# sara-nl/2D-VQ-AE-2

Hardware: AMD Instinct MI355X
Metric: patches/sec (VQAE.forward: encoder -> VQ -> decoder) (higher is better)
Workload: dtype f32; 1 GPU; BASELINE configs[1] (cfg B): batch 256/GPU of 256x256x3 fp32 -> 32x32 codes, K=256, D=128, full forward; global_batch=256, parallelism=patch-sharded x1

## Files before the change

### 2d-vq-ae-2_amd/_lib.py

```python
import ctypes
import os
from ctypes import POINTER, Structure, c_char_p, c_double, c_float, c_int, c_int64, c_size_t, c_void_p

_HERE = os.path.dirname(os.path.abspath(__file__))
LIB_PATH = os.environ.get("VQAE_HIP_LIB") or os.path.join(_HERE, "libvqae_hip.so")

LAYOUT_NHWC, LAYOUT_NCHW = 0, 1
IDX_I64, IDX_U8, IDX_U16, IDX_I32 = 0, 1, 2, 3
PAD_NONE, PAD_CIRCULAR, PAD_ZEROS = 0, 1, 2
PRE_NONE, PRE_BIAS, PRE_BIAS_ELU_BIAS, PRE_CHANNEL_GATE = 0, 1, 2, 3
ACT_NONE, ACT_ELU, ACT_SILU = 0, 1, 2
DW_SAME, DW_DOWN, DW_UP = 0, 1, 2
MBT_ROWS, MBT_FIN_LANES = 256, 64
BLOCK_FIXUP, BLOCK_MBCONV = 0, 1
DT_F32, DT_BF16, DT_F16 = 0, 1, 2
MAX_PIXEL_LEVEL = 6
METRIC_NAMES = ("mse", "huber", "psnr", "ssim", "pred_min", "pred_max", "target_min", "target_max")
CLS_STATS_NAMES = ("tp", "fp", "fn", "tn", "n_valid", "loss_sum")
CE_STATS_K, CE_WEIGHT_SUM, CE_NLL_SUM, CE_SMOOTH_SUM, CE_N_BAD = 20, 16, 17, 18, 19
DTYPES = {"f32": DT_F32, "fp32": DT_F32, "float32": DT_F32, "bf16": DT_BF16, "bfloat16": DT_BF16,
          "f16": DT_F16, "fp16": DT_F16, "float16": DT_F16, "half": DT_F16}


def dtype_code(dt):
    if dt is None:
        return DT_F32
    if isinstance(dt, int):
        return dt
    name = str(dt).replace("torch.", "")
    try:
        return DTYPES[name]
    except KeyError:
        raise AssertionError(f"unsupported compute dtype {dt}")


class VqaeHipError(RuntimeError):
    pass


class ConvArgs(Structure):
    _fields_ = [("batch", c_int), ("in_h", c_int), ("in_w", c_int), ("cin", c_int), ("cout", c_int),
                ("ksize", c_int), ("stride", c_int), ("pad", c_int), ("pad_mode", c_int),
                ("pre_mode", c_int), ("pre_a", c_float), ("pre_b", c_float),
                ("has_scale", c_int), ("has_bias_s", c_int), ("has_act", c_int),
                ("scale", c_float), ("bias_s", c_float), ("act_a", c_float), ("act_b", c_float), ("dtype", c_int)]


class Config(Structure):
    _fields_ = [("in_channels", c_int), ("stem", c_int), ("n_down", c_int), ("n_pre", c_int), ("n_post", c_int),
                ("n_enc", c_int), ("num_embeddings", c_int), ("projection_dim", c_int),
                ("commitment_cost", c_float), ("compute_dtype", c_int),
                ("block_kind", c_int), ("expand_ratio", c_int), ("se_divisor", c_int), ("bn_eps", c_float)]


class Tensor(Structure):
    _fields_ = [("name", c_char_p), ("data", c_void_p), ("numel", c_int64)]


OPTIM_KINDS = {"adam": 0, "adamw": 1, "lamb": 2}
OPTIM_CHUNK, OPTIM_SMALL = 4096, 64


class ClassifierOptimConfig(Structure):
    _fields_ = [("kind", c_int), ("lr", c_double), ("beta1", c_double), ("beta2", c_double), ("eps", c_double),
                ("weight_decay", c_double), ("sam_rho", c_double), ("sam_adaptive", c_int)]


SYMBOLS = {
    "vqae_last_error": (c_char_p, []),
    "vqae_build_info": (c_char_p, []),
    "vqae_vq_workspace_bytes": (c_size_t, [c_int64, c_int, c_int]),
    "vqae_vq_forward_f32": (c_int, [c_void_p, c_void_p, c_int64, c_int, c_int, c_float, c_void_p, c_int, c_void_p,
                                    c_void_p, c_void_p, c_void_p, c_void_p]),
    "vqae_vq_forward_p_f32": (c_int, [c_void_p, c_void_p, c_int64, c_int, c_int, c_int, c_float, c_void_p, c_int, c_void_p,
                                      c_void_p, c_void_p, c_void_p, c_void_p]),
    "vqae_vq_projected_workspace_bytes": (c_size_t, [c_int64]),
    "vqae_vq_projected_f32": (c_int, [c_void_p, c_void_p, c_void_p, c_void_p, c_void_p, c_void_p, c_int64, c_int, c_int, c_int,
                                      c_float, c_int, c_void_p, c_int, c_void_p, c_void_p, c_void_p, c_void_p, c_void_p, c_void_p]),
    "vqae_vq_backward_f32": (c_int, [c_void_p, c_void_p, c_void_p, c_void_p, c_float, c_int64, c_int, c_void_p, c_void_p]),
    "vqae_vq_projected_backward_workspace_bytes": (c_size_t, [c_int64, c_int]),
    "vqae_vq_projected_backward_f32": (c_int, [c_void_p, c_void_p, c_void_p, c_void_p, c_void_p, c_void_p, c_void_p, c_int64,
                                               c_int, c_int, c_float, c_void_p, c_void_p, c_void_p, c_void_p, c_void_p,
                                               c_void_p, c_void_p]),
    "vqae_embed_code_f32": (c_int, [c_void_p, c_int, c_void_p, c_int64, c_int, c_int, c_void_p, c_void_p]),
    "vqae_vq_code_stats_f32": (c_int, [c_void_p, c_void_p, c_int, c_int64, c_int, c_int, c_void_p, c_void_p, c_void_p]),
    "vqae_vq_ema_update_f32": (c_int, [c_void_p, c_void_p, c_void_p, c_void_p, c_void_p, c_int, c_int, c_double, c_double,
                                       c_void_p, c_void_p]),
    "vqae_conv_packed_floats": (c_size_t, [c_int, c_int, c_int]),
    "vqae_conv_pack_weight_f32": (c_int, [c_void_p, c_int, c_int, c_int, c_void_p, c_void_p]),
    "vqae_conv2d_f32": (c_int, [POINTER(ConvArgs), c_void_p, c_void_p, c_void_p, c_void_p, c_void_p, c_void_p]),
    "vqae_conv2d_gated_f32": (c_int, [POINTER(ConvArgs), c_void_p, c_void_p, c_void_p, c_void_p, c_void_p, c_void_p,
                                      c_void_p]),
    "vqae_dw_partial_floats": (c_size_t, [c_int, c_int, c_int, c_int]),
    "vqae_dwconv_f32": (c_int, [c_void_p, c_void_p, c_void_p, c_int, c_int, c_int, c_int, c_int, c_int, c_void_p,
                                c_void_p, c_void_p]),
    "vqae_se_gate_f32": (c_int, [c_void_p, c_int, c_int, c_int, c_int, c_void_p, c_void_p, c_int, c_void_p, c_void_p,
                                 c_void_p, c_void_p]),
    "vqae_pixel_shuffle2_f32": (c_int, [c_void_p, c_int, c_int, c_int, c_int, c_void_p, c_void_p]),
    "vqae_fixup_same_supported": (c_int, [c_int, c_int, c_int]),
    "vqae_fixup_same_block_f32": (c_int, [c_void_p, c_void_p, c_void_p, c_void_p, c_void_p, c_int, c_int, c_int, c_int,
                                          POINTER(c_float), c_int, c_void_p]),
    "vqae_round_inplace_f32": (c_int, [c_void_p, c_int64, c_int, c_void_p]),
    "vqae_conv3x3_direct_f32": (c_int, [c_void_p, c_void_p, POINTER(c_float), POINTER(c_float), c_void_p, c_void_p,
                                        c_int, c_int, c_int, c_int, c_int, c_void_p, c_int, c_void_p]),
    "vqae_bicubic_up2_f32": (c_int, [c_void_p, c_int, c_int, c_int, c_int, c_float, c_void_p, c_void_p]),
    "vqae_nchw_to_nhwc_f32": (c_int, [c_void_p, c_int, c_int, c_int, c_int, c_void_p, c_void_p]),
    "vqae_nhwc_to_nchw_f32": (c_int, [c_void_p, c_int, c_int, c_int, c_int, c_void_p, c_void_p]),
    "vqae_label_maxpool_u8": (c_int, [c_void_p, c_int, c_int, c_int, c_int, c_void_p, c_void_p]),
    "vqae_stitch_tiles": (c_int, [c_void_p, c_int, c_void_p, c_int, c_int, c_int, c_void_p, c_int, c_int, c_int,
                                  c_void_p]),
    "vqae_unstitch_tiles": (c_int, [c_void_p, c_int, c_void_p, c_int, c_int, c_int, c_void_p, c_int, c_int, c_int,
                                    c_void_p]),
    "vqae_pixels_u8": (c_int, [c_void_p, c_int, c_int, c_int, c_int, c_void_p, POINTER(c_float), POINTER(c_float), c_void_p,
                               c_int, c_int, c_void_p]),
    "vqae_pixels_u8_level": (c_int, [c_void_p, c_int, c_int, c_int, c_int, c_int, c_void_p, POINTER(c_float), POINTER(c_float),
                                     c_void_p, c_int, c_int, c_void_p]),
    "vqae_cut_pixels_u8": (c_int, [c_void_p, c_int, c_int, c_int, c_void_p, c_int, c_int, c_int, c_int, c_int, c_int, c_void_p,
                                   c_void_p]),
    "vqae_pool_labels_u8": (c_int, [c_void_p, c_int, c_int, c_int, c_int, c_int, c_int, c_void_p, c_int, c_int, c_void_p]),
    "vqae_create": (c_int, [POINTER(Config), POINTER(Tensor), c_int, POINTER(c_void_p)]),
    "vqae_destroy": (None, [c_void_p]),
    "vqae_reserve": (c_int, [c_void_p, c_int, c_int, c_int]),
    "vqae_set_codebook": (c_int, [c_void_p, c_void_p]),
    "vqae_encode": (c_int, [c_void_p, c_void_p, c_int, c_int, c_int, c_int, c_void_p, c_int, c_void_p, c_void_p,
                            c_void_p]),
    "vqae_encode_u8": (c_int, [c_void_p, c_void_p, c_int, c_int, c_int, c_void_p, c_int, c_void_p, c_int, c_void_p,
                               c_void_p]),
    "vqae_encode_features": (c_int, [c_void_p, c_void_p, c_int, c_int, c_int, c_int, c_void_p, c_void_p]),
    "vqae_decode": (c_int, [c_void_p, c_void_p, c_int, c_int, c_int, c_int, c_void_p, c_void_p]),
    "vqae_decode_indices": (c_int, [c_void_p, c_void_p, c_int, c_int, c_int, c_int, c_int, c_void_p, c_void_p]),
    "vqae_decode_indices_u8": (c_int, [c_void_p, c_void_p, c_int, c_int, c_int, c_int, c_void_p, c_void_p, c_int, c_int,
                                       c_void_p]),
    "vqae_decode_indices_u8_levels": (c_int, [c_void_p, c_void_p, c_int, c_int, c_int, c_int, c_void_p, c_int, POINTER(c_int),
                                              POINTER(c_void_p), POINTER(c_int), POINTER(c_int), c_void_p]),
    "vqae_forward": (c_int, [c_void_p, c_void_p, c_int, c_int, c_int, c_int, c_void_p, c_void_p, c_int, c_void_p,
                             c_void_p]),
    "vqae_block_count": (c_int, [c_void_p, c_int]),
    "vqae_run_blocks": (c_int, [c_void_p, c_int, c_int, c_int, c_void_p, c_int, c_int, c_int, c_void_p, POINTER(c_int),
                                POINTER(c_int), c_void_p]),
    "vqae_block_route": (c_char_p, [c_void_p, c_int, c_int, c_int, c_int, c_int, c_int]),
    "vqae_recon_metrics_workspace_bytes": (c_size_t, [c_int, c_int, c_int, c_int]),
    "vqae_recon_metrics_f32": (c_int, [c_void_p, c_void_p, c_void_p, POINTER(c_float), POINTER(c_float), c_int, c_int, c_int,
                                       c_int, c_int, c_float, c_void_p, c_void_p, c_void_p]),
    "vqae_classifier_create": (c_int, [c_int, c_int, c_int, c_int, POINTER(Tensor), c_int, POINTER(c_void_p)]),
    "vqae_classifier_destroy": (None, [c_void_p]),
    "vqae_classifier_workspace_bytes": (c_size_t, [c_void_p, c_int, c_int, c_int]),
    "vqae_classifier_forward": (c_int, [c_void_p, c_void_p, c_int, c_int, c_int, c_int, c_void_p, c_void_p, c_void_p, c_float,
                                        c_void_p, c_void_p, c_void_p]),
    "vqae_classifier_update": (c_int, [c_void_p, POINTER(Tensor), c_int]),
    "vqae_classifier_grad_floats": (c_size_t, [c_void_p]),
    "vqae_classifier_train_workspace_bytes": (c_size_t, [c_void_p, c_int, c_int, c_int]),
    "vqae_classifier_loss_grad": (c_int, [c_void_p, c_void_p, c_int, c_int, c_int, c_int, c_void_p, c_void_p, c_float, c_int,
                                          c_void_p, c_void_p, c_void_p, c_void_p, c_void_p]),
    "vqae_classifier_optim_create": (c_int, [c_void_p, POINTER(ClassifierOptimConfig), POINTER(c_void_p)]),
    "vqae_classifier_optim_destroy": (None, [c_void_p]),
    "vqae_classifier_optim_set": (c_int, [c_void_p, POINTER(ClassifierOptimConfig)]),
    "vqae_classifier_optim_step": (c_int, [c_void_p, c_void_p, c_void_p]),
    "vqae_classifier_optim_sam_first": (c_int, [c_void_p, c_void_p, c_void_p]),
    "vqae_classifier_download": (c_int, [c_void_p, POINTER(c_void_p), c_void_p]),
    "vqae_classifier_image_floats": (c_size_t, [c_void_p]),
    "vqae_classifier_image": (c_int, [c_void_p, c_void_p, c_void_p]),
    "vqae_classifier_optim_export": (c_int, [c_void_p, c_void_p, c_void_p, POINTER(c_int64), c_void_p]),
    "vqae_classifier_optim_import": (c_int, [c_void_p, c_void_p, c_void_p, c_int64, c_void_p]),
    "vqae_classifier_ce_workspace_bytes": (c_size_t, [c_void_p, c_int, c_int, c_int]),
    "vqae_classifier_forward_ce": (c_int, [c_void_p, c_void_p, c_int, c_int, c_int, c_int, c_void_p, c_void_p, c_void_p, c_void_p,
                                           POINTER(c_float), c_float, c_void_p, c_void_p, c_void_p]),
    "vqae_classifier_ce_train_workspace_bytes": (c_size_t, [c_void_p, c_int, c_int, c_int]),
    "vqae_classifier_loss_grad_ce": (c_int, [c_void_p, c_void_p, c_int, c_int, c_int, c_int, c_void_p, POINTER(c_float), c_float,
                                             c_int, c_void_p, c_void_p, c_void_p, c_void_p, c_void_p]),
    "vqae_classifier_optim_create_ce": (c_int, [c_void_p, POINTER(ClassifierOptimConfig), POINTER(c_void_p)]),
    "vqae_optim_create": (c_int, [c_int, POINTER(c_int64), POINTER(c_int), c_int, POINTER(ClassifierOptimConfig),
                                  POINTER(c_void_p)]),
    "vqae_optim_destroy": (None, [c_void_p]),
    "vqae_optim_set": (c_int, [c_void_p, POINTER(ClassifierOptimConfig)]),
    "vqae_optim_step": (c_int, [c_void_p, POINTER(c_void_p), POINTER(c_void_p), c_void_p]),
    "vqae_optim_sam_first": (c_int, [c_void_p, POINTER(c_void_p), POINTER(c_void_p), c_void_p]),
    "vqae_optim_export": (c_int, [c_void_p, c_void_p, c_void_p, POINTER(c_int64), c_void_p]),
    "vqae_optim_import": (c_int, [c_void_p, c_void_p, c_void_p, POINTER(c_int64), c_void_p]),
    "vqae_fixup_train_workspace_bytes": (c_size_t, [c_int64]),
    "vqae_fixup_act_f32": (c_int, [c_void_p, c_void_p, c_void_p, c_int, c_int, c_int, c_int, c_int, c_int, c_void_p, c_void_p]),
    "vqae_fixup_act_backward_f32": (c_int, [c_void_p, c_void_p, c_void_p, c_int, c_int, c_int, c_int, c_int, c_int, c_void_p,
                                            c_void_p, c_void_p, c_void_p, c_void_p]),
    "vqae_fixup_out_f32": (c_int, [c_void_p, c_void_p, c_void_p, c_void_p, c_void_p, c_int64, c_void_p, c_void_p]),
    "vqae_fixup_out_backward_f32": (c_int, [c_void_p, c_void_p, c_void_p, c_int64, c_void_p, c_void_p, c_void_p, c_void_p,
                                            c_void_p, c_void_p]),
    "vqae_fixup_act_io": (c_int, [c_void_p, c_int, c_void_p, c_void_p, c_int, c_int, c_int, c_int, c_int, c_int, c_void_p, c_int,
                                  c_void_p]),
# ... 93 lines not shown
```

### 2d-vq-ae-2_amd/csrc/misc_kernels.hip

```cpp
#include "kernels.h"
#include "mfma.h"

namespace {


template <int CIN, int COUT>
__global__ __launch_bounds__(256)
void conv3x3_direct_kernel(const void* __restrict__ xin, int x_kind, Norm3 nrm, const float* __restrict__ w,
                           const float* __restrict__ bias, int B, int H, int W, float* __restrict__ y, int y_nchw,
                           int dt) {
    __shared__ float ws[9 * CIN * COUT + COUT];
    for (int i = threadIdx.x; i < 9 * CIN * COUT; i += 256) {
        const int co = i % COUT, ci = (i / COUT) % CIN, tap = i / (COUT * CIN);
        ws[i] = vqae::round_dt(w[((int64_t)co * CIN + ci) * 9 + tap], dt);
    }
    for (int i = threadIdx.x; i < COUT; i += 256) ws[9 * CIN * COUT + i] = vqae::round_dt(bias[i], dt);
    __syncthreads();

    const int64_t npix = (int64_t)B * H * W;
    const int64_t pix = (int64_t)blockIdx.x * 256 + threadIdx.x;
    if (pix >= npix) return;
    const int hw = H * W;
    const int b = (int)(pix / hw), rem = (int)(pix - (int64_t)b * hw);
    const int oy = rem / W, ox = rem - oy * W;
// ... 151 lines not shown
    if (i >= (int64_t)B * O * O) return;
    const int ox = (int)(i % O), oy = (int)((i / O) % O), b = (int)(i / ((int64_t)O * O));
    const int y0 = (oy * H) / O, y1 = ((oy + 1) * H + O - 1) / O;
    const int x0 = (ox * W) / O, x1 = ((ox + 1) * W + O - 1) / O;
    uint8_t m = 0;
    for (int yy = y0; yy < y1; ++yy)
        for (int xx = x0; xx < x1; ++xx) {
            const uint8_t v = lab[((int64_t)b * H + yy) * W + xx];
            m = v > m ? v : m;
        }
    y[i] = m;
}

template <typename TI, typename TO>
__global__ __launch_bounds__(256)
void stitch_kernel(const TI* __restrict__ tiles, const int32_t* __restrict__ rc, int64_t total, int th, int tw,
                   TO* __restrict__ grid, int gh, int gw) {
    const int64_t i = (int64_t)blockIdx.x * 256 + threadIdx.x;
    if (i >= total) return;
    const int x = (int)(i % tw), yy = (int)((i / tw) % th);
    const int64_t t = i / ((int64_t)tw * th);
    const int r = rc[2 * t], c = rc[2 * t + 1];
    const int64_t gy = (int64_t)r * th + yy, gx = (int64_t)c * tw + x;
    if (gy < gh && gx < gw) grid[gy * gw + gx] = (TO)tiles[i];
}

template <int CIN>
__global__ __launch_bounds__(256)
void ostem_rb_kernel(const float* __restrict__ x, const float* __restrict__ w, const float* __restrict__ bias, int B, int H, int W,
                     float* __restrict__ y, int y_nchw) {
    constexpr int QN = CIN / 4;
    typedef float f32x4_t __attribute__((ext_vector_type(4)));
    const int q = threadIdx.x % QN;
    f32x4_t wr[9][3];
#pragma unroll
    for (int tap = 0; tap < 9; ++tap)
#pragma unroll
        for (int co = 0; co < 3; ++co)
#pragma unroll
            for (int e = 0; e < 4; ++e) wr[tap][co][e] = w[((int64_t)co * CIN + 4 * q + e) * 9 + tap];
    const float b0 = bias[0], b1 = bias[1], b2 = bias[2];
    const int hw = H * W;
    const int64_t npix = (int64_t)B * hw;
    const int64_t stride = (int64_t)gridDim.x * (256 / QN);
    const int64_t trips = (npix + stride - 1) / stride;
    int64_t pix = (int64_t)blockIdx.x * (256 / QN) + threadIdx.x / QN;
    for (int64_t t = 0; t < trips; ++t, pix += stride) {
        const bool live = pix < npix;
        const int64_t pc = live ? pix : npix - 1;
        const int b = (int)(pc / hw), rem = (int)(pc - (int64_t)b * hw);
        const int oy = rem / W, ox = rem - oy * W;
        float a0 = 0.f, a1 = 0.f, a2 = 0.f;
#pragma unroll
        for (int tap = 0; tap < 9; ++tap) {
            const int iy = oy + tap / 3 - 1, ix = ox + tap % 3 - 1;
            const bool ok = iy >= 0 && iy < H && ix >= 0 && ix < W;
            const int64_t src = ((int64_t)b * hw + (ok ? (int64_t)iy * W + ix : rem)) * CIN + 4 * q;
            f32x4_t v = *reinterpret_cast<const f32x4_t*>(x + src);
            if (!ok) v = (f32x4_t){0.f, 0.f, 0.f, 0.f};
#pragma unroll
            for (int e = 0; e < 4; ++e) {
                a0 = __builtin_fmaf(v[e], wr[tap][0][e], a0);
                a1 = __builtin_fmaf(v[e], wr[tap][1][e], a1);
                a2 = __builtin_fmaf(v[e], wr[tap][2][e], a2);
            }
        }
#pragma unroll
        for (int off = 1; off < QN; off <<= 1) {
            a0 += __shfl_xor(a0, off);
            a1 += __shfl_xor(a1, off);
            a2 += __shfl_xor(a2, off);
        }
        if (live && q == 0) {
            a0 += b0; a1 += b1; a2 += b2;
            if (y_nchw) {
                y[((int64_t)b * 3 + 0) * hw + rem] = a0;
                y[((int64_t)b * 3 + 1) * hw + rem] = a1;
                y[((int64_t)b * 3 + 2) * hw + rem] = a2;
            } else {
                y[pix * 3 + 0] = a0; y[pix * 3 + 1] = a1; y[pix * 3 + 2] = a2;
            }
        }
    }
}

template <int CIN, int COUT>
int launch_direct(const void* x, int x_kind, const Norm3& nrm, const float* w, const float* bias, int B, int H, int W,
                  float* y, int y_nchw, int dt, hipStream_t stream) {
    const int64_t npix = (int64_t)B * H * W;
    conv3x3_direct_kernel<CIN, COUT><<<(unsigned)vqae::ceil_div(npix, 256), 256, 0, stream>>>(
        x, x_kind, nrm, w, bias, B, H, W, y, y_nchw, dt);
    VQAE_LAUNCH_CHECK();
    return VQAE_OK;
}

template <typename TI>
int stitch_out(const TI* tiles, const int32_t* rc, int64_t total, int th, int tw, void* grid, int gdt, int gh, int gw,
               hipStream_t stream) {
    const unsigned g = (unsigned)vqae::ceil_div(total, 256);
    switch (gdt) {
        case VQAE_IDX_I64: stitch_kernel<TI, int64_t><<<g, 256, 0, stream>>>(tiles, rc, total, th, tw, (int64_t*)grid, gh, gw); break;
        case VQAE_IDX_U8: stitch_kernel<TI, uint8_t><<<g, 256, 0, stream>>>(tiles, rc, total, th, tw, (uint8_t*)grid, gh, gw); break;
        case VQAE_IDX_U16: stitch_kernel<TI, uint16_t><<<g, 256, 0, stream>>>(tiles, rc, total, th, tw, (uint16_t*)grid, gh, gw); break;
        case VQAE_IDX_I32: stitch_kernel<TI, int32_t><<<g, 256, 0, stream>>>(tiles, rc, total, th, tw, (int32_t*)grid, gh, gw); break;
        default: return vqae::fail(VQAE_ERR_INVALID, "stitch: bad grid dtype %d", gdt);
    }
    VQAE_LAUNCH_CHECK();
    return VQAE_OK;
}


struct SmallK {
    const float* __restrict__ x;
    const float* __restrict__ w;
    const float* __restrict__ bias_vec;
    const float* residual;
    float* y;
    int H, W, Ho, Wo, cout;
    int64_t M;
    int pre_mode, has_scale, has_bias_s, has_act, dt;
    float pre_a, pre_b, scale, bias_s, act_a, act_b;
};

template <int KS>
__global__ __launch_bounds__(256)
void conv_small_k_kernel(const SmallK p) {
    constexpr int K = KS * KS * 8;
    __shared__ __attribute__((aligned(16))) float Wl[K * 64];
    const int cg4 = p.cout >> 2;
    for (int j = threadIdx.x; j < K * p.cout; j += 256) Wl[j] = p.w[(int64_t)(j % p.cout) * K + j / p.cout];
    __syncthreads();
    const int64_t i = (int64_t)blockIdx.x * 256 + threadIdx.x;
    if (i >= p.M * cg4) return;
    const int cg = (int)(i % cg4);
    const int64_t m = i / cg4;
    const int ox = (int)(m % p.Wo);
    const int64_t t = m / p.Wo;
    const int oy = (int)(t % p.Ho);
    const int64_t b = t / p.Ho;
    float v[K];
#pragma unroll
    for (int tap = 0; tap < KS * KS; ++tap) {
        const float4* src = reinterpret_cast<const float4*>(
            p.x + (((b * p.H + (int64_t)oy * KS + tap / KS) * p.W) + (int64_t)ox * KS + tap % KS) * 8);
        const float4 a = src[0], c = src[1];
        v[tap * 8 + 0] = a.x; v[tap * 8 + 1] = a.y; v[tap * 8 + 2] = a.z; v[tap * 8 + 3] = a.w;
        v[tap * 8 + 4] = c.x; v[tap * 8 + 5] = c.y; v[tap * 8 + 6] = c.z; v[tap * 8 + 7] = c.w;
    }
#pragma unroll
    for (int k = 0; k < K; ++k) {
        if (p.pre_mode != VQAE_PRE_NONE) {
            v[k] = v[k] + p.pre_a;
            if (p.pre_mode == VQAE_PRE_BIAS_ELU_BIAS) v[k] = vqae::elu_act(v[k]) + p.pre_b;
        }
        v[k] = vqae::round_dt(v[k], p.dt);
    }
    float out[4] = {0.f, 0.f, 0.f, 0.f};
#pragma unroll
    for (int k = 0; k < K; ++k) {
        const float4 wv = *reinterpret_cast<const float4*>(Wl + k * p.cout + 4 * cg);
        out[0] = __builtin_fmaf(v[k], wv.x, out[0]); out[1] = __builtin_fmaf(v[k], wv.y, out[1]);
        out[2] = __builtin_fmaf(v[k], wv.z, out[2]); out[3] = __builtin_fmaf(v[k], wv.w, out[3]);
    }
#pragma unroll
    for (int e = 0; e < 4; ++e) {
        float acc = out[e];
        if (p.bias_vec) acc = acc + p.bias_vec[4 * cg + e];
        acc = vqae::round_dt(acc, p.dt);
        if (p.has_scale) { acc = acc * p.scale; acc = acc + p.bias_s; }
        else if (p.has_bias_s) { acc = acc + p.bias_s; }
        out[e] = acc;
    }
    const int64_t o = m * p.cout + 4 * cg;
    if (p.residual) {
        const float4 r = *reinterpret_cast<const float4*>(p.residual + o);
        out[0] += r.x; out[1] += r.y; out[2] += r.z; out[3] += r.w;
    }
    if (p.has_act == VQAE_ACT_SILU) {
#pragma unroll
        for (int e = 0; e < 4; ++e) out[e] = out[e] / (1.0f + expf(-out[e]));
    } else if (p.has_act) {
#pragma unroll
        for (int e = 0; e < 4; ++e) out[e] = vqae::elu_act(out[e] + p.act_a) + p.act_b;
    }
    *reinterpret_cast<float4*>(p.y + o) = make_float4(out[0], out[1], out[2], out[3]);
}

}

namespace vqae {
bool conv_small_k_supported(const vqae_conv_args* a) {
    return a->cin == 8 && a->pad == 0 && a->ksize == a->stride && (a->ksize == 1 || a->ksize == 2) && a->cout % 4 == 0 &&
           a->cout <= 64 && a->pre_mode <= VQAE_PRE_BIAS_ELU_BIAS && a->in_h % a->ksize == 0 && a->in_w % a->ksize == 0;
}

int conv_small_k(const vqae_conv_args* a, const float* x, const float* w, const float* bias_vec, const float* residual,
                 float* y, hipStream_t stream) {
    SmallK p;
    p.x = x; p.w = w; p.bias_vec = bias_vec; p.residual = residual; p.y = y;
    p.H = a->in_h; p.W = a->in_w; p.Ho = a->in_h / a->ksize; p.Wo = a->in_w / a->ksize; p.cout = a->cout;
    p.M = (int64_t)a->batch * p.Ho * p.Wo;
    p.pre_mode = a->pre_mode; p.has_scale = a->has_scale; p.has_bias_s = a->has_bias_s; p.has_act = a->has_act; p.dt = a->dtype;
    p.pre_a = a->pre_a; p.pre_b = a->pre_b; p.scale = a->scale; p.bias_s = a->bias_s; p.act_a = a->act_a; p.act_b = a->act_b;
    const int64_t threads = p.M * (a->cout / 4);
    if (threads == 0) return VQAE_OK;
    VQAE_REQUIRE(ceil_div(threads, 256) < (1ll << 31), VQAE_ERR_UNSUPPORTED, "conv_small_k: too many pixels");
    const unsigned grid = (unsigned)ceil_div(threads, 256);
    if (a->ksize == 1) conv_small_k_kernel<1><<<grid, 256, 0, stream>>>(p);
    else conv_small_k_kernel<2><<<grid, 256, 0, stream>>>(p);
    VQAE_LAUNCH_CHECK();
    return VQAE_OK;
}

int conv3x3_direct(const void* x, int x_kind, const float* mean255, const float* inv_std255, const float* w,
                   const float* bias, int B, int H, int W, int cin, int cout, float* y, int y_nchw, int dt,
                   hipStream_t stream) {
    Norm3 nrm;
    for (int i = 0; i < 4; ++i) {
        nrm.mean[i] = (mean255 && i < 3) ? mean255[i] : 0.f;
        nrm.inv[i] = (inv_std255 && i < 3) ? inv_std255[i] : 1.f;
    }
    VQAE_REQUIRE(x && w && bias && y, VQAE_ERR_INVALID, "conv3x3_direct: null pointer");
    VQAE_REQUIRE(x_kind != 2 || cin == 3, VQAE_ERR_UNSUPPORTED, "conv3x3_direct: uint8 input needs cin == 3");
    if ((int64_t)B * H * W == 0) return VQAE_OK;
    static const bool no_rb = env_int("VQAE_NO_STEM_RB", 0) != 0;
    if (!no_rb && dt == VQAE_DT_F32) {
        if (cout == 3 && x_kind == 0 && (cin == 8 || cin == 16 || cin == 32)) {
            const int64_t npix = (int64_t)B * H * W;
            const unsigned grid = (unsigned)std::min<int64_t>(vqae::ceil_div(npix, 256 / (cin / 4)), 256 * 12);
            if (cin == 8) ostem_rb_kernel<8><<<grid, 256, 0, stream>>>((const float*)x, w, bias, B, H, W, y, y_nchw);
            else if (cin == 16) ostem_rb_kernel<16><<<grid, 256, 0, stream>>>((const float*)x, w, bias, B, H, W, y, y_nchw);
            else ostem_rb_kernel<32><<<grid, 256, 0, stream>>>((const float*)x, w, bias, B, H, W, y, y_nchw);
            VQAE_LAUNCH_CHECK();
            return VQAE_OK;
        }
    }
#define VQAE_DIRECT_CASE(CI, CO) \
    if (cin == CI && cout == CO) return launch_direct<CI, CO>(x, x_kind, nrm, w, bias, B, H, W, y, y_nchw, dt, stream);
    VQAE_DIRECT_CASE(3, 4) VQAE_DIRECT_CASE(3, 8) VQAE_DIRECT_CASE(3, 16) VQAE_DIRECT_CASE(3, 32) VQAE_DIRECT_CASE(3, 64)
    VQAE_DIRECT_CASE(4, 3) VQAE_DIRECT_CASE(8, 3) VQAE_DIRECT_CASE(16, 3) VQAE_DIRECT_CASE(32, 3) VQAE_DIRECT_CASE(64, 3)
#undef VQAE_DIRECT_CASE
    return fail(VQAE_ERR_UNSUPPORTED, "conv3x3_direct: unsupported channel pair %d -> %d", cin, cout);
}
}

extern "C" int vqae_conv3x3_direct_f32(const float* x, const uint8_t* x_u8, const float* mean255, const float* inv_std255,
                                       const float* w, const float* bias, int B, int H, int W, int cin, int cout,
                                       float* y, int dtype, void* stream) {
    VQAE_REQUIRE(dtype >= VQAE_DT_F32 && dtype <= VQAE_DT_F16, VQAE_ERR_INVALID, "conv3x3_direct: dtype %d", dtype);
    static const bool no16 = vqae::env_int("VQAE_NO_STEM16", 0) != 0;
    const int c0 = cin == 3 ? cout : (cout == 3 ? cin : 0);
    if (!no16 && dtype != VQAE_DT_F32 && c0 && (cin == 3) != (cout == 3) && vqae::stem16_supported(c0, H, W, dtype) && (cin == 3 || x)) {
        VQAE_REQUIRE((x || x_u8) && w && bias && y, VQAE_ERR_INVALID, "conv3x3_direct: null pointer");
        void* wbuf = nullptr;
        VQAE_HIP_CHECK(hipMallocAsync(&wbuf, vqae::stem16_weight_bytes(32), (hipStream_t)stream));
        int rc = vqae::stem16_pack_weight(w, cout, cin, dtype, wbuf, (hipStream_t)stream);
        if (rc == VQAE_OK)
            rc = cin == 3 ? vqae::istem16(x_u8 ? (const void*)x_u8 : (const void*)x, x_u8 ? 2 : 0, mean255, inv_std255, wbuf, bias, B, H, W,
                                          cout, y, dtype, (hipStream_t)stream)
                          : vqae::ostem16(x, wbuf, bias, B, H, W, cin, y, 0, dtype, (hipStream_t)stream);
        const hipError_t fe = hipFreeAsync(wbuf, (hipStream_t)stream);
        if (rc == VQAE_OK && fe != hipSuccess) return vqae::fail(VQAE_ERR_HIP, "conv3x3_direct: hipFreeAsync: %s", hipGetErrorString(fe));
        return rc;
    }
    if (x_u8)
        return vqae::conv3x3_direct(x_u8, 2, mean255, inv_std255, w, bias, B, H, W, cin, cout, y, 0, dtype, (hipStream_t)stream);
    return vqae::conv3x3_direct(x, 0, nullptr, nullptr, w, bias, B, H, W, cin, cout, y, 0, dtype, (hipStream_t)stream);
}

namespace {
__global__ void round_inplace_kernel(float* __restrict__ x, int64_t n, int dt) {
    const int64_t i = (int64_t)blockIdx.x * 256 + threadIdx.x;
    if (i < n) x[i] = vqae::round_dt(x[i], dt);
}
}

extern "C" int vqae_round_inplace_f32(float* x, int64_t n, int dtype, void* stream) {
    VQAE_REQUIRE(dtype >= VQAE_DT_F32 && dtype <= VQAE_DT_F16, VQAE_ERR_INVALID, "round_inplace: dtype %d", dtype);
    if (n == 0 || dtype == VQAE_DT_F32) return VQAE_OK;
    VQAE_REQUIRE(x, VQAE_ERR_INVALID, "round_inplace: null pointer");
    round_inplace_kernel<<<(unsigned)vqae::ceil_div(n, 256), 256, 0, (hipStream_t)stream>>>(x, n, dtype);
    VQAE_LAUNCH_CHECK();
    return VQAE_OK;
}

extern "C" int vqae_bicubic_up2_f32(const float* x, int B, int H, int W, int C, float pre_bias, float* y, void* stream_) {
    hipStream_t stream = (hipStream_t)stream_;
    VQAE_REQUIRE(x && y, VQAE_ERR_INVALID, "bicubic_up2: null pointer");
    VQAE_REQUIRE(C % 4 == 0, VQAE_ERR_UNSUPPORTED, "bicubic_up2: channels %d must be a multiple of 4", C);
    if ((int64_t)B * H * W == 0) return VQAE_OK;
    const int64_t total = (int64_t)B * (H + 1) * (W + 1) * (C / 4);
    const unsigned grid = (unsigned)std::min<int64_t>(vqae::ceil_div(total, 256), 256 * 64);
    bicubic_up2_kernel<<<grid, 256, 0, stream>>>((const float4*)x, B, H, W, C / 4, pre_bias, (float4*)y);
    VQAE_LAUNCH_CHECK();
    return VQAE_OK;
}

static int transpose_batched(const float* x, int B, int R, int S, float* y, hipStream_t stream) {
    if ((int64_t)B * R * S == 0) return VQAE_OK;
    VQAE_REQUIRE(B <= 65535, VQAE_ERR_UNSUPPORTED, "transpose: batch %d > 65535", B);
    dim3 grid((unsigned)vqae::ceil_div(S, 32), (unsigned)vqae::ceil_div(R, 32), (unsigned)B);
    transpose_kernel<<<grid, 256, 0, stream>>>(x, R, S, y);
    VQAE_LAUNCH_CHECK();
    return VQAE_OK;
}

extern "C" int vqae_nchw_to_nhwc_f32(const float* x, int B, int C, int H, int W, float* y, void* stream) {
    VQAE_REQUIRE(x && y, VQAE_ERR_INVALID, "nchw_to_nhwc: null pointer");
    return transpose_batched(x, B, C, H * W, y, (hipStream_t)stream);
}

extern "C" int vqae_nhwc_to_nchw_f32(const float* x, int B, int C, int H, int W, float* y, void* stream) {
    VQAE_REQUIRE(x && y, VQAE_ERR_INVALID, "nhwc_to_nchw: null pointer");
    return transpose_batched(x, B, H * W, C, y, (hipStream_t)stream);
}

extern "C" int vqae_label_maxpool_u8(const uint8_t* lab, int B, int H, int W, int O, uint8_t* y, void* stream_) {
    hipStream_t stream = (hipStream_t)stream_;
    VQAE_REQUIRE(lab && y, VQAE_ERR_INVALID, "label_maxpool: null pointer");
    VQAE_REQUIRE(O >= 1 && O <= H && O <= W, VQAE_ERR_INVALID, "label_maxpool: output %d larger than input", O);
    const int64_t total = (int64_t)B * O * O;
    if (total == 0) return VQAE_OK;
    label_maxpool_kernel<<<(unsigned)vqae::ceil_div(total, 256), 256, 0, stream>>>(lab, B, H, W, O, y);
    VQAE_LAUNCH_CHECK();
    return VQAE_OK;
}

extern "C" int vqae_stitch_tiles(const void* tiles, int idx_dtype, const int32_t* rc, int n_tiles, int th, int tw,
                                 void* grid, int grid_dtype, int gh, int gw, void* stream_) {
    hipStream_t stream = (hipStream_t)stream_;
    VQAE_REQUIRE(tiles && rc && grid, VQAE_ERR_INVALID, "stitch: null pointer");
    const int64_t total = (int64_t)n_tiles * th * tw;
    if (total == 0) return VQAE_OK;
    switch (idx_dtype) {
        case VQAE_IDX_I64: return stitch_out((const int64_t*)tiles, rc, total, th, tw, grid, grid_dtype, gh, gw, stream);
        case VQAE_IDX_U8: return stitch_out((const uint8_t*)tiles, rc, total, th, tw, grid, grid_dtype, gh, gw, stream);
        case VQAE_IDX_U16: return stitch_out((const uint16_t*)tiles, rc, total, th, tw, grid, grid_dtype, gh, gw, stream);
        case VQAE_IDX_I32: return stitch_out((const int32_t*)tiles, rc, total, th, tw, grid, grid_dtype, gh, gw, stream);
        default: return vqae::fail(VQAE_ERR_INVALID, "stitch: bad tile dtype %d", idx_dtype);
    }
}
```

### 2d-vq-ae-2_amd/ops.py

```python
import ctypes
import functools
import types

import torch

from . import _lib as L

_IDX_DTYPES = {torch.int64: L.IDX_I64, torch.uint8: L.IDX_U8, torch.int32: L.IDX_I32}
if hasattr(torch, "uint16"):
    _IDX_DTYPES[torch.uint16] = L.IDX_U16


MEAN = (0.7279, 0.5955, 0.7762)
STD = (0.2419, 0.3083, 0.1741)


def _stream():
    return ctypes.c_void_p(torch.cuda.current_stream().cuda_stream)


def _need_gpu(*ts):
    for t in ts:
        if t is not None and not t.is_cuda:
            raise L.VqaeHipError("libvqae_hip ops need tensors in HBM (device='cuda'); there is no CPU fallback")
# ... 46 lines not shown
    B, H, W, cin = x.shape
    a = L.ConvArgs()
    a.batch, a.in_h, a.in_w, a.cin, a.cout = B, H, W, cin, cout
    a.ksize, a.stride, a.pad, a.pad_mode = ksize, stride, pad, pad_mode
    a.dtype = L.dtype_code(dtype)
    if pre is not None:
        if len(pre) == 1:
            a.pre_mode, a.pre_a = L.PRE_BIAS, float(pre[0])
        else:
            a.pre_mode, a.pre_a, a.pre_b = L.PRE_BIAS_ELU_BIAS, float(pre[0]), float(pre[1])
    if isinstance(act, str):
        assert act == "silu", act
        a.has_act = L.ACT_SILU
    elif act is not None:
        a.has_act, a.act_a, a.act_b = L.ACT_ELU, float(act[0]), float(act[1])
    if scale_bias is not None:
        a.has_scale, a.scale, a.bias_s = 1, float(scale_bias[0]), float(scale_bias[1])
    elif bias_s is not None:
        a.has_bias_s, a.bias_s = 1, float(bias_s)
    Ho = (H + 2 * pad - ksize) // stride + 1
    Wo = (W + 2 * pad - ksize) // stride + 1
    if out is None:
        out = torch.empty((B, Ho, Wo, cout), dtype=torch.float32, device=x.device)
    if gate is not None:
        assert pre is None and tuple(gate.shape) == (B, cin), (pre, gate.shape)
        _need_gpu(gate)
        a.pre_mode = L.PRE_CHANNEL_GATE
        L.check(L.lib().vqae_conv2d_gated_f32(ctypes.byref(a), _p(x), _p(gate.contiguous()), _p(w_packed), _p(bias_vec),
                                              _p(residual), _p(out), _stream()))
        return out
    L.check(L.lib().vqae_conv2d_f32(ctypes.byref(a), _p(x), _p(w_packed), _p(bias_vec), _p(residual), _p(out),
                                    _stream()))
    return out


def dwconv(x, w_taps, bias=None, mode=L.DW_SAME, silu=False, want_partial=False):
    _need_gpu(x, w_taps)
    x = x.contiguous()
    B, H, W, C = x.shape
    Ho, Wo = {L.DW_SAME: (H, W), L.DW_DOWN: (H // 2, W // 2), L.DW_UP: (2 * H, 2 * W)}[mode]
    y = torch.empty((B, Ho, Wo, C), dtype=torch.float32, device=x.device)
    part = None
    if want_partial:
        part = torch.empty(int(L.lib().vqae_dw_partial_floats(B, Ho, Wo, C)), dtype=torch.float32, device=x.device)
    L.check(L.lib().vqae_dwconv_f32(_p(x), _p(w_taps.contiguous()), _p(bias), B, H, W, C, mode, int(silu), _p(y), _p(part),
                                    _stream()))
    return (y, part) if want_partial else y


def se_gate(partial, batch, out_h, out_w, fc0_w, fc0_b, fc2_w, fc2_b):
    _need_gpu(partial, fc0_w, fc0_b, fc2_w, fc2_b)
    hidden, C = fc0_w.shape
    gate = torch.empty((batch, C), dtype=torch.float32, device=partial.device)
    L.check(L.lib().vqae_se_gate_f32(_p(partial), batch, out_h, out_w, C, _p(fc0_w.contiguous()), _p(fc0_b.contiguous()),
                                     hidden, _p(fc2_w.contiguous()), _p(fc2_b.contiguous()), _p(gate), _stream()))
    return gate


def pixel_shuffle2(x, c):
    _need_gpu(x)
    x = x.contiguous()
    B, H, W, c4 = x.shape
    assert c4 == 4 * c
    y = torch.empty((B, 2 * H, 2 * W, c), dtype=torch.float32, device=x.device)
    L.check(L.lib().vqae_pixel_shuffle2_f32(_p(x), B, H, W, c, _p(y), _stream()))
    return y


def fixup_same_supported(c, h, w):
    return bool(L.lib().vqae_fixup_same_supported(c, h, w))


def fixup_same_block(x, w1p, w2p, w3p, scalars8, dtype=None):
    _need_gpu(x, w1p, w2p, w3p)
    x = x.contiguous()
    B, H, W, C = x.shape
    y = torch.empty_like(x)
    sc = (ctypes.c_float * 8)(*[float(v) for v in scalars8])
    L.check(L.lib().vqae_fixup_same_block_f32(_p(x), _p(y), _p(w1p), _p(w2p), _p(w3p), B, H, W, C, sc,
                                              L.dtype_code(dtype), _stream()))
    return y


def conv3x3_direct(x, w, bias, x_u8=None, mean255=None, inv_std255=None, dtype=None):
    src = x if x_u8 is None else x_u8
    _need_gpu(src, w, bias)
    src = src.contiguous()
    B, H, W, cin = src.shape
    cout = w.shape[0]
    y = torch.empty((B, H, W, cout), dtype=torch.float32, device=src.device)
    m = (ctypes.c_float * 3)(*mean255) if mean255 is not None else None
    s = (ctypes.c_float * 3)(*inv_std255) if inv_std255 is not None else None
    L.check(L.lib().vqae_conv3x3_direct_f32(_p(x) if x_u8 is None else None, _p(x_u8) if x_u8 is not None else None,
                                            m, s, _p(w.contiguous()), _p(bias.contiguous()), B, H, W, cin, cout,
                                            _p(y), L.dtype_code(dtype), _stream()))
    return y


def bicubic_up2(x, pre_bias=0.0):
    _need_gpu(x)
    x = x.contiguous()
    B, H, W, C = x.shape
    y = torch.empty((B, 2 * H, 2 * W, C), dtype=torch.float32, device=x.device)
    L.check(L.lib().vqae_bicubic_up2_f32(_p(x), B, H, W, C, float(pre_bias), _p(y), _stream()))
    return y


def _scalar(p):
    if p is None:
        return None
    _need_gpu(p)
    return p.detach().reshape(-1)[:1].float().contiguous()


def _train_ws(n, dev):
    return torch.empty(L.lib().vqae_fixup_train_workspace_bytes(int(n)), dtype=torch.uint8, device=dev)


_IO_DTYPES = {torch.float32: L.DT_F32, torch.bfloat16: L.DT_BF16, torch.float16: L.DT_F16}


def _need_f32(who, **tensors):
    for name, t in tensors.items():
        assert t is None or t.dtype == torch.float32, f"{who}: {name} is {t.dtype}; the fp32 op takes fp32 tensors (see {who}_io)"


def _io_code(who, name, dtype):
    try:
        return _IO_DTYPES[dtype]
    except KeyError:
        raise AssertionError(f"{who}: {name} is {dtype}; fp32, bf16 and f16 are taken")


def fixup_act(x, a, b, halo=0):
    _need_gpu(x)
    x = x.contiguous()
    B, H, W, C = x.shape
    y = torch.empty((B, H + 2 * halo, W + 2 * halo, C), dtype=torch.float32, device=x.device)
    L.check(L.lib().vqae_fixup_act_f32(_p(x), _p(_scalar(a)), _p(_scalar(b)), int(a is not None), int(halo), B, H, W, C, _p(y),
                                       _stream()))
    return y


def fixup_act_backward(g, x, a, halo=0, act=True):
    _need_f32("fixup_act_backward", g=g, x=x if act else None)
    _need_gpu(g)
    g = g.contiguous()
    B, H, W, C = g.shape[0], g.shape[1] - 2 * halo, g.shape[2] - 2 * halo, g.shape[3]
    dev = g.device
    g_b = torch.empty(1, dtype=torch.float32, device=dev)
    ws = _train_ws(g.numel(), dev)
    if not act:
        L.check(L.lib().vqae_fixup_act_backward_f32(_p(g), None, None, 0, 0, B, H, W, C, None, None, _p(g_b), _p(ws), _stream()))
        return g, None, g_b
    x = x.contiguous()
    assert tuple(x.shape) == (B, H, W, C), (x.shape, g.shape)
    g_x = torch.empty((B, H, W, C), dtype=torch.float32, device=dev)
    g_a = torch.empty(1, dtype=torch.float32, device=dev)
    L.check(L.lib().vqae_fixup_act_backward_f32(_p(g), _p(x), _p(_scalar(a)), 1, int(halo), B, H, W, C, _p(g_x), _p(g_a), _p(g_b),
                                                _p(ws), _stream()))
    return g_x, g_a, g_b


def fixup_out(t, skip, scale, bias4, bias1d=None):
    _need_gpu(t, skip)
    t, skip = t.contiguous(), skip.contiguous()
    assert t.shape == skip.shape, (t.shape, skip.shape)
    y = torch.empty_like(t)
    L.check(L.lib().vqae_fixup_out_f32(_p(t), _p(skip), _p(_scalar(scale)), _p(_scalar(bias4)), _p(_scalar(bias1d)), t.numel(),
                                       _p(y), _stream()))
    return y

# ... 855 lines not shown
```

### include/vqae_hip.h

```cpp
#ifndef VQAE_HIP_H
#define VQAE_HIP_H

#include <stddef.h>
#include <stdint.h>

#ifdef __cplusplus
extern "C" {
#endif

typedef enum vqae_status {
    VQAE_OK = 0,
    VQAE_ERR_INVALID = -1,
    VQAE_ERR_UNSUPPORTED = -2,
    VQAE_ERR_HIP = -3,
    VQAE_ERR_NOMEM = -4,
    VQAE_ERR_NOT_FOUND = -5,
    VQAE_ERR_VALUE = -6
} vqae_status;

enum { VQAE_LAYOUT_NHWC = 0, VQAE_LAYOUT_NCHW = 1 };
enum { VQAE_DT_F32 = 0, VQAE_DT_BF16 = 1, VQAE_DT_F16 = 2 };
enum { VQAE_IDX_I64 = 0, VQAE_IDX_U8 = 1, VQAE_IDX_U16 = 2, VQAE_IDX_I32 = 3 };

const char* vqae_last_error(void);
// ... 1 lines not shown


size_t vqae_vq_workspace_bytes(int64_t n_rows, int n_codes, int dim);

int vqae_vq_forward_f32(const float* z_dev, const float* embed_dev, int64_t n_rows, int n_codes, int dim,
                        float commitment_cost, void* idx_dev, int idx_dtype, float* q_dev, float* loss_dev,
                        float* margin_dev, void* workspace_dev, void* stream);

int vqae_vq_forward_p_f32(const float* z_dev, const float* embed_dev, int64_t n_rows, int n_codes, int dim, int p,
                          float commitment_cost, void* idx_dev, int idx_dtype, float* q_dev, float* loss_dev,
                          float* margin_dev, void* workspace_dev, void* stream);

size_t vqae_vq_projected_workspace_bytes(int64_t n_rows);
int vqae_vq_projected_f32(const float* x_dev, const float* wt_in_dev, const float* b_in_dev, const float* embed_dev,
                          const float* w_out_dev, const float* b_out_dev, int64_t n_rows, int channels, int projection_dim,
                          int n_codes, float commitment_cost, int dtype, void* idx_dev, int idx_dtype, float* out_dev,
                          float* z_dev, float* loss_dev, float* margin_dev, void* workspace_dev, void* stream);

int vqae_vq_backward_f32(const float* g_q_dev, const float* z_dev, const float* q_dev, const float* g_loss_dev,
                         float commitment_cost, int64_t n_rows, int dim, float* g_z_dev, void* stream);

size_t vqae_vq_projected_backward_workspace_bytes(int64_t n_rows, int channels);
int vqae_vq_projected_backward_f32(const float* g_out_dev, const float* x_dev, const float* z_dev, const float* q_dev,
                                   const float* g_loss_dev, const float* wt_in_dev, const float* w_out_dev, int64_t n_rows,
                                   int channels, int projection_dim, float commitment_cost, float* g_x_dev,
                                   float* g_w_in_dev, float* g_b_in_dev, float* g_w_out_dev, float* g_b_out_dev,
                                   void* workspace_dev, void* stream);

int vqae_embed_code_f32(const void* idx_dev, int idx_dtype, const float* embed_dev, int64_t n_rows, int n_codes,
                        int dim, float* out_dev, void* stream);

int vqae_vq_code_stats_f32(const float* z_dev, const void* idx_dev, int idx_dtype, int64_t n_rows, int n_codes,
                           int dim, float* counts_dev, float* dw_dev, void* stream);
int vqae_vq_ema_update_f32(float* embed_dev, float* embed_avg_dev, float* cluster_size_dev, const float* counts_dev,
                           const float* dw_dev, int n_codes, int dim, double decay, double laplace_alpha,
                           void* workspace_dev , void* stream);


enum { VQAE_PAD_NONE = 0, VQAE_PAD_CIRCULAR = 1, VQAE_PAD_ZEROS = 2 };
enum { VQAE_PRE_NONE = 0, VQAE_PRE_BIAS = 1, VQAE_PRE_BIAS_ELU_BIAS = 2, VQAE_PRE_CHANNEL_GATE = 3 };
enum { VQAE_ACT_NONE = 0, VQAE_ACT_ELU = 1, VQAE_ACT_SILU = 2 };

size_t vqae_conv_packed_floats(int cout, int cin, int ksize);
int vqae_conv_pack_weight_f32(const float* w_oihw_dev, int cout, int cin, int ksize, float* packed_dev,
                              void* stream);

typedef struct vqae_conv_args {
    int batch, in_h, in_w, cin, cout;
    int ksize;
    int stride;
    int pad;
    int pad_mode;
    int pre_mode;
    float pre_a, pre_b;
    int has_scale, has_bias_s, has_act;
    float scale, bias_s, act_a, act_b;
    int dtype;
} vqae_conv_args;

int vqae_conv2d_f32(const vqae_conv_args* a, const float* x_dev, const float* w_packed_dev,
                    const float* bias_vec_dev, const float* residual_dev, float* y_dev, void* stream);

int vqae_conv2d_gated_f32(const vqae_conv_args* a, const float* x_dev, const float* gate_dev, const float* w_packed_dev,
                          const float* bias_vec_dev, const float* residual_dev, float* y_dev, void* stream);

enum { VQAE_DW_SAME = 0, VQAE_DW_DOWN = 1, VQAE_DW_UP = 2 };
size_t vqae_dw_partial_floats(int batch, int out_h, int out_w, int channels);
int vqae_dwconv_f32(const float* x_dev, const float* w_taps_dev, const float* bias_dev, int batch, int h, int w,
                    int channels, int mode, int silu, float* y_dev, float* partial_dev, void* stream);
int vqae_se_gate_f32(const float* partial_dev, int batch, int out_h, int out_w, int channels, const float* fc0_w_dev,
                     const float* fc0_b_dev, int hidden, const float* fc2_w_dev, const float* fc2_b_dev, float* gate_dev,
                     void* stream);
int vqae_pixel_shuffle2_f32(const float* x_dev, int batch, int h, int w, int c, float* y_dev, void* stream);

int vqae_fixup_same_supported(int c, int h, int w);
int vqae_fixup_same_block_f32(const float* x_dev, float* y_dev, const float* w1_packed_dev, const float* w2_packed_dev,
                              const float* w3_packed_dev, int batch, int h, int w, int c, const float* scalars8,
                              int dtype , void* stream);
int vqae_round_inplace_f32(float* x_dev, int64_t n, int dtype, void* stream);

int vqae_conv3x3_direct_f32(const float* x_dev, const uint8_t* x_u8_dev, const float* mean255, const float* inv_std255,
                            const float* w_oihw_dev, const float* bias_dev, int batch, int h, int w, int cin,
                            int cout, float* y_dev, int dtype , void* stream);

int vqae_bicubic_up2_f32(const float* x_dev, int batch, int h, int w, int c, float pre_bias, float* y_dev,
                         void* stream);

int vqae_nchw_to_nhwc_f32(const float* x_dev, int batch, int c, int h, int w, float* y_dev, void* stream);
int vqae_nhwc_to_nchw_f32(const float* x_dev, int batch, int c, int h, int w, float* y_dev, void* stream);

int vqae_label_maxpool_u8(const uint8_t* labels_dev, int batch, int h, int w, int out, uint8_t* y_dev, void* stream);

int vqae_stitch_tiles(const void* tiles_dev, int idx_dtype, const int32_t* rc_dev, int n_tiles, int th, int tw,
                      void* grid_dev, int grid_dtype, int grid_h, int grid_w, void* stream);

int vqae_unstitch_tiles(const void* grid_dev, int grid_dtype, const int32_t* rc_dev, int n_tiles, int th, int tw,
                        void* tiles_dev, int idx_dtype, int grid_h, int grid_w, void* stream);

int vqae_pixels_u8(const float* x_dev, int layout, int batch, int h, int w, const int32_t* rc_dev, const float* mean255,
                   const float* std255, uint8_t* out_dev, int canvas_h, int canvas_w, void* stream);

enum { VQAE_MAX_PIXEL_LEVEL = 6 };
int vqae_pixels_u8_level(const float* x_dev, int layout, int batch, int h, int w, int level, const int32_t* rc_dev,
                         const float* mean255, const float* std255, uint8_t* out_dev, int canvas_h, int canvas_w,
                         void* stream);

int vqae_cut_pixels_u8(const uint8_t* canvas_dev, int canvas_h, int canvas_w, int ch, const int32_t* rc_dev, int n_tiles, int h,
                       int w, int y0, int x0, int level, uint8_t* tiles_dev, void* stream);

int vqae_pool_labels_u8(const uint8_t* mask_dev, int mask_h, int mask_w, int y0, int x0, int win_h, int win_w, uint8_t* out_dev,
                        int out_h, int out_w, void* stream);

typedef struct vqae_config {
    int in_channels;
    int stem;
    int n_down;
    int n_pre, n_post;
    int n_enc;
    int num_embeddings;
    int projection_dim;
    float commitment_cost;
    int compute_dtype;
    int block_kind;
    int expand_ratio;
    int se_divisor;
    float bn_eps;
} vqae_config;
enum { VQAE_BLOCK_FIXUP = 0, VQAE_BLOCK_MBCONV = 1 };

typedef struct vqae_tensor {
    const char* name;
    const float* data;
    int64_t numel;
} vqae_tensor;

typedef struct vqae_handle vqae_handle;

int vqae_create(const vqae_config* cfg, const vqae_tensor* tensors, int n_tensors, vqae_handle** out);
void vqae_destroy(vqae_handle* h);
int vqae_reserve(vqae_handle* h, int max_batch, int in_h, int in_w);
int vqae_set_codebook(vqae_handle* h, const float* embed_host);

int vqae_encode(vqae_handle* h, const float* x_dev, int batch, int in_h, int in_w, int layout, void* idx_dev,
                int idx_dtype, float* q_dev, float* loss_dev, void* stream);
int vqae_encode_u8(vqae_handle* h, const uint8_t* x_u8_dev, int batch, int in_h, int in_w, void* idx_dev,
                   int idx_dtype, float* q_dev, int q_layout, float* loss_dev, void* stream);
int vqae_encode_features(vqae_handle* h, const float* x_dev, int batch, int in_h, int in_w, int layout,
                         float* z_dev, void* stream);
int vqae_decode(vqae_handle* h, const float* q_dev, int batch, int q_h, int q_w, int layout, float* out_dev,
                void* stream);
int vqae_decode_indices(vqae_handle* h, const void* idx_dev, int idx_dtype, int batch, int q_h, int q_w, int layout,
                        float* out_dev, void* stream);
int vqae_decode_indices_u8(vqae_handle* h, const void* idx_dev, int idx_dtype, int batch, int q_h, int q_w,
                           const int32_t* rc_dev, uint8_t* canvas_dev, int canvas_h, int canvas_w, void* stream);
int vqae_decode_indices_u8_levels(vqae_handle* h, const void* idx_dev, int idx_dtype, int batch, int q_h, int q_w,
                                  const int32_t* rc_dev, int n_levels, const int* levels, uint8_t* const* canvases,
                                  const int* canvas_h, const int* canvas_w, void* stream);
int vqae_forward(vqae_handle* h, const float* x_dev, int batch, int in_h, int in_w, int layout, float* out_dev,
                 void* idx_dev, int idx_dtype, float* loss_dev, void* stream);

int vqae_block_count(const vqae_handle* h, int side);
int vqae_run_blocks(vqae_handle* h, int side, int first, int count, const float* x_dev, int batch, int in_h, int in_w,
                    float* y_dev, int* out_h, int* out_w, void* stream);
const char* vqae_block_route(const vqae_handle* h, int side, int index, int chained, int batch, int in_h, int in_w);

double vqae_flops_per_patch(const vqae_handle* h, int in_h, int in_w, int encoder, int decoder);
// ... 204 lines not shown
```

Baseline: 4581 patches/s.

## Add LDS-tiled persistent output-stem conv kernel with prefetch and NCHW-output entry

Adds a tiled 3x3 output-stem convolution (cout=3) that stages a halo window of the input into LDS per tile. It uses a persistent grid that prefetches the next tile into registers while computing the current one. Weights are double-buffered in registers across channel groups. It replaces the previous per-pixel row-batched kernel by default, aiming to cut redundant global reads of neighbouring pixels. It also adds a C/Python entry point that writes NCHW output directly, which the Python wrapper can use to skip a separate transpose.

```diff
diff --git a/2d-vq-ae-2_amd/_lib.py b/2d-vq-ae-2_amd/_lib.py
--- a/2d-vq-ae-2_amd/_lib.py
+++ b/2d-vq-ae-2_amd/_lib.py
@@ -103,6 +103,8 @@
     "vqae_round_inplace_f32": (c_int, [c_void_p, c_int64, c_int, c_void_p]),
     "vqae_conv3x3_direct_f32": (c_int, [c_void_p, c_void_p, POINTER(c_float), POINTER(c_float), c_void_p, c_void_p,
                                         c_int, c_int, c_int, c_int, c_int, c_void_p, c_int, c_void_p]),
+    "vqae_conv3x3_direct_layout_f32": (c_int, [c_void_p, c_void_p, c_void_p, c_int, c_int, c_int, c_int, c_int, c_void_p,
+                                               c_int, c_void_p]),
     "vqae_bicubic_up2_f32": (c_int, [c_void_p, c_int, c_int, c_int, c_int, c_float, c_void_p, c_void_p]),
     "vqae_nchw_to_nhwc_f32": (c_int, [c_void_p, c_int, c_int, c_int, c_int, c_void_p, c_void_p]),
     "vqae_nhwc_to_nchw_f32": (c_int, [c_void_p, c_int, c_int, c_int, c_int, c_void_p, c_void_p]),
diff --git a/2d-vq-ae-2_amd/csrc/misc_kernels.hip b/2d-vq-ae-2_amd/csrc/misc_kernels.hip
--- a/2d-vq-ae-2_amd/csrc/misc_kernels.hip
+++ b/2d-vq-ae-2_amd/csrc/misc_kernels.hip
@@ -257,6 +257,132 @@
             }
         }
     }
+}
+
+template <int CIN, int TR>
+struct OstemTile {
+    static constexpr int QN = CIN / 4, TC = 64, WC = TC + 2, NP = (TR + 2) * WC;
+    static constexpr int PS = NP + ((8 / QN) - NP % 8 + 8) % 8;
+    static constexpr int NT = 64 * TR;
+    static constexpr int NITEM = NP * QN, NIT = (NITEM + NT - 1) / NT;
+    static constexpr int LDS_BYTES = QN * PS * 16;
+};
+
+template <int CIN, int TR>
+__global__ __launch_bounds__(64 * TR)
+void ostem_tiled_kernel(const float* __restrict__ x, const float* __restrict__ w, const float* __restrict__ bias, int B, int H, int W,
+                        int tiles_x, int tiles_y, float* __restrict__ y, int y_nchw) {
+    typedef OstemTile<CIN, TR> T;
+    constexpr int QN = T::QN, WC = T::WC, PS = T::PS, NT = T::NT, NIT = T::NIT;
+    typedef float f32x4_t __attribute__((ext_vector_type(4)));
+    __shared__ __attribute__((aligned(16))) float win[T::LDS_BYTES / 4];
+    const int tid = threadIdx.x;
+    int it_rc[NIT], it_off[NIT], it_lds[NIT];
+#pragma unroll
+    for (int i = 0; i < NIT; ++i) {
+        int idx = tid + NT * i;
+        idx = idx < T::NITEM ? idx : T::NITEM - 1;
+        const int wp = idx / QN, q = idx % QN;
+        it_rc[i] = (wp / WC) << 16 | (wp % WC);
+        it_off[i] = ((wp / WC) * W + wp % WC) * CIN + 4 * q;
+        it_lds[i] = (q * PS + wp) * 4;
+    }
+    const int hw = H * W;
+    const int n_tiles = B * tiles_x * tiles_y;
+    const int row = tid >> 6, col = tid & 63;
+    const float* base = win + (row * WC + col) * 4;
+
+    f32x4_t v[NIT];
+    auto fetch = [&](int tile) {
+        const int txi = tile % tiles_x, tyi = (tile / tiles_x) % tiles_y;
+        const int b = tile / (tiles_x * tiles_y);
+        const int gy0 = TR * tyi - 1, gx0 = T::TC * txi - 1;
+        const float* org = x + ((int64_t)b * hw + (int64_t)gy0 * W + gx0) * CIN;
+#pragma unroll
+        for (int i = 0; i < NIT; ++i) {
+            const int gy = gy0 + (it_rc[i] >> 16), gx = gx0 + (it_rc[i] & 0xffff);
+            f32x4_t t = {0.f, 0.f, 0.f, 0.f};
+            if (((unsigned)gy < (unsigned)H) & ((unsigned)gx < (unsigned)W)) t = *reinterpret_cast<const f32x4_t*>(org + it_off[i]);
+            v[i] = t;
+        }
+    };
+    int tile = blockIdx.x;
+    if (tile < n_tiles) fetch(tile);
+    for (; tile < n_tiles; tile += gridDim.x) {
+        vqae::lds_barrier();
+#pragma unroll
+        for (int i = 0; i < NIT; ++i)
+            if (T::NITEM % NT == 0 || tid + NT * i < T::NITEM) *reinterpret_cast<f32x4_t*>(win + it_lds[i]) = v[i];
+        vqae::lds_barrier();
+        const int txi = tile % tiles_x, tyi = (tile / tiles_x) % tiles_y;
+        const int b = tile / (tiles_x * tiles_y);
+        if (tile + (int)gridDim.x < n_tiles) fetch(tile + gridDim.x);
+
+        float s[QN * 3];
+        float wk[2][36];
+        auto wload = [&](int k, float tie) -> float {
+            int wz;
+            asm volatile("s_mov_b32 %0, 0" : "=s"(wz), "+v"(tie));
+            const float* wq = w + wz + ((k % 3) * CIN + 4 * (k / 3)) * 9;
+#pragma unroll
+            for (int j = 0; j < 36; ++j) wk[k & 1][j] = wq[j];
+            return tie;
+        };
+        (void)wload(0, 0.f);
+        f32x4_t in[9];
+#pragma unroll
+        for (int k = 0; k < QN * 3; ++k) {
+            if (k % 3 == 0) {
+#pragma unroll
+                for (int tap = 0; tap < 9; ++tap)
+                    in[tap] = *reinterpret_cast<const f32x4_t*>(base + ((k / 3) * PS + (tap / 3) * WC + tap % 3) * 4);
+            }
+            if (k + 1 < QN * 3) {
+                if (k >= 1) s[k - 1] = wload(k + 1, s[k - 1]); else (void)wload(k + 1, 0.f);
+            }
+            float a = 0.f;
+#pragma unroll
+            for (int tap = 0; tap < 9; ++tap)
+#pragma unroll
+                for (int e = 0; e < 4; ++e) a = __builtin_fmaf(in[tap][e], wk[k & 1][e * 9 + tap], a);
+            s[k] = a;
+        }
+        const int oy = TR * tyi + row, ox = T::TC * txi + col;
+        if (oy < H && ox < W) {
+            float o[3];
+#pragma unroll
+            for (int co = 0; co < 3; ++co) {
+                float r;
+                if constexpr (QN == 2) r = s[co] + s[3 + co];
+                else if constexpr (QN == 4) r = (s[co] + s[3 + co]) + (s[6 + co] + s[9 + co]);
+                else r = ((s[co] + s[3 + co]) + (s[6 + co] + s[9 + co])) + ((s[12 + co] + s[15 + co]) + (s[18 + co] + s[21 + co]));
+                o[co] = r + bias[co];
+            }
+            const int rem = oy * W + ox;
+            if (y_nchw) {
+                float* dst = y + (int64_t)b * 3 * hw + rem;
+                dst[0] = o[0]; dst[hw] = o[1]; dst[2 * (int64_t)hw] = o[2];
+            } else {
+                float* dst = y + ((int64_t)b * hw + rem) * 3;
+                dst[0] = o[0]; dst[1] = o[1]; dst[2] = o[2];
+            }
+        }
+    }
+}
+
+template <int CIN, int TR>
+int launch_ostem_tiled(const float* x, const float* w, const float* bias, int B, int H, int W, float* y, int y_nchw,
+                       hipStream_t stream) {
+    typedef OstemTile<CIN, TR> T;
+    static_assert(4 * T::LDS_BYTES <= 160 * 1024, "four workgroups per CU");
+    const int tiles_x = (int)vqae::ceil_div(W, T::TC), tiles_y = (int)vqae::ceil_div(H, TR);
+    const int64_t n_tiles = (int64_t)B * tiles_x * tiles_y;
+    VQAE_REQUIRE(n_tiles < (1ll << 30) && (int64_t)H * W < (1ll << 29) && (int64_t)W * CIN * (TR + 2) < (1ll << 31), VQAE_ERR_UNSUPPORTED,
+                 "out_stem: image too large for 32-bit tile and window offsets");
+    const unsigned grid = (unsigned)std::min<int64_t>(n_tiles, 256 * 12);
+    ostem_tiled_kernel<CIN, TR><<<grid, T::NT, 0, stream>>>(x, w, bias, B, H, W, tiles_x, tiles_y, y, y_nchw);
+    VQAE_LAUNCH_CHECK();
+    return VQAE_OK;
 }
 
 template <int CIN, int COUT>
@@ -401,6 +527,11 @@
     static const bool no_rb = env_int("VQAE_NO_STEM_RB", 0) != 0;
     if (!no_rb && dt == VQAE_DT_F32) {
         if (cout == 3 && x_kind == 0 && (cin == 8 || cin == 16 || cin == 32)) {
+            if (env_int("VQAE_NO_OSTEM_TILED", 0) == 0) {
+                if (cin == 8) return launch_ostem_tiled<8, 4>((const float*)x, w, bias, B, H, W, y, y_nchw, stream);
+                if (cin == 16) return launch_ostem_tiled<16, 4>((const float*)x, w, bias, B, H, W, y, y_nchw, stream);
+                return launch_ostem_tiled<32, 2>((const float*)x, w, bias, B, H, W, y, y_nchw, stream);
+            }
             const int64_t npix = (int64_t)B * H * W;
             const unsigned grid = (unsigned)std::min<int64_t>(vqae::ceil_div(npix, 256 / (cin / 4)), 256 * 12);
             if (cin == 8) ostem_rb_kernel<8><<<grid, 256, 0, stream>>>((const float*)x, w, bias, B, H, W, y, y_nchw);
@@ -443,6 +574,13 @@
     return vqae::conv3x3_direct(x, 0, nullptr, nullptr, w, bias, B, H, W, cin, cout, y, 0, dtype, (hipStream_t)stream);
 }
 
+extern "C" int vqae_conv3x3_direct_layout_f32(const float* x, const float* w, const float* bias, int B, int H, int W, int cin,
+                                              int cout, float* y, int y_layout, void* stream) {
+    VQAE_REQUIRE(y_layout == VQAE_LAYOUT_NHWC || y_layout == VQAE_LAYOUT_NCHW, VQAE_ERR_INVALID, "conv3x3_direct: layout %d", y_layout);
+    return vqae::conv3x3_direct(x, 0, nullptr, nullptr, w, bias, B, H, W, cin, cout, y, y_layout == VQAE_LAYOUT_NCHW ? 1 : 0,
+                                VQAE_DT_F32, (hipStream_t)stream);
+}
+
 namespace {
 __global__ void round_inplace_kernel(float* __restrict__ x, int64_t n, int dt) {
     const int64_t i = (int64_t)blockIdx.x * 256 + threadIdx.x;
diff --git a/2d-vq-ae-2_amd/ops.py b/2d-vq-ae-2_amd/ops.py
--- a/2d-vq-ae-2_amd/ops.py
+++ b/2d-vq-ae-2_amd/ops.py
@@ -152,12 +152,19 @@
     return y
 
 
-def conv3x3_direct(x, w, bias, x_u8=None, mean255=None, inv_std255=None, dtype=None):
+def conv3x3_direct(x, w, bias, x_u8=None, mean255=None, inv_std255=None, dtype=None, nchw_out=False):
     src = x if x_u8 is None else x_u8
     _need_gpu(src, w, bias)
     src = src.contiguous()
     B, H, W, cin = src.shape
     cout = w.shape[0]
+    if nchw_out:
+        if x_u8 is not None or L.dtype_code(dtype) != L.dtype_code(None):
+            raise ValueError("conv3x3_direct: nchw_out takes an fp32 input in the fp32 mode")
+        y = torch.empty((B, cout, H, W), dtype=torch.float32, device=src.device)
+        L.check(L.lib().vqae_conv3x3_direct_layout_f32(_p(src), _p(w.contiguous()), _p(bias.contiguous()), B, H, W, cin, cout,
+                                                       _p(y), 1, _stream()))
+        return y
     y = torch.empty((B, H, W, cout), dtype=torch.float32, device=src.device)
     m = (ctypes.c_float * 3)(*mean255) if mean255 is not None else None
     s = (ctypes.c_float * 3)(*inv_std255) if inv_std255 is not None else None
diff --git a/include/vqae_hip.h b/include/vqae_hip.h
--- a/include/vqae_hip.h
+++ b/include/vqae_hip.h
@@ -107,6 +107,8 @@
 int vqae_conv3x3_direct_f32(const float* x_dev, const uint8_t* x_u8_dev, const float* mean255, const float* inv_std255,
                             const float* w_oihw_dev, const float* bias_dev, int batch, int h, int w, int cin,
                             int cout, float* y_dev, int dtype , void* stream);
+int vqae_conv3x3_direct_layout_f32(const float* x_dev, const float* w_oihw_dev, const float* bias_dev, int batch, int h, int w,
+                                   int cin, int cout, float* y_dev, int y_layout , void* stream);
 
 int vqae_bicubic_up2_f32(const float* x_dev, int batch, int h, int w, int c, float pre_bias, float* y_dev,
                          void* stream);
```

Result: no change. 4609 patches/s (median of 6 runs) (+0.6%).
